# GuanLab/seekmer

Measured on AMD Instinct MI355X. Metric: paired reads/sec mapped+quantified, higher is better.
Workload: dtype u64+f64; 1 GPU; configs[1]: synthetic ~190k-tx index (stand-in for ENSEMBL GRCh38 cDNA), 10000000 2x100bp synthetic pairs per GPU, map+classes+EM to the reference stop rule; transcripts=190402, kmer_slots=134217728, units_per_gpu=10000000, read_len=100, paired=True, classes=851072, class_map_rows=4208693, parallelism=reads sharded x1, RCCL all-reduce f64[T] per EM step, rccl_ranks=0

## Files before the change

seekmer_amd/csrc/skm_abi.hip:

```cpp
#include "../../include/seekmer_hip.h"
#include "skm_kernels.h"
#include "skm_pool.h"
#include "skm_bias.h"
#include "skm_bias_weights.h"

#include <dlfcn.h>
#include <algorithm>
#include <cmath>
#include <cstdarg>
#include <cstdio>
#include <cstdlib>
#include <cstring>
#include <chrono>
#include <condition_variable>
#include <atomic>
#include <deque>
#include <functional>
#include <map>
#include <memory>
#include <unordered_map>
#include <mutex>
#include <thread>
#include <numeric>
#include <string>
// ... 3697 lines not shown
        aligned = q->pinned[32];
        q->n_total_reduced = true;
        if (const char *v = getenv("SKM_TEST_ALIGNED_GLOBAL")) aligned += strtoull(v, nullptr, 10);
    }
    q->n_total = (double)aligned;
    HIP_TRY(hipMemcpyAsync(q->x1.p, lengths, n_tx * 8, hipMemcpyHostToDevice, q->stream));
    if (m->use_length_weights)
        launch_effective_lengths_weights(m->length_weights.p, 1, q->x1.p, n_tx, q->eff_len.p, q->stream);
    else
        launch_effective_lengths(fld.p, q->x1.p, n_tx, q->eff_len.p, q->stream);
    if (q->comm ? aligned == 0 : C == 0) {
        if (effective_lengths)
            HIP_TRY(hipMemcpyAsync(effective_lengths, q->eff_len.p, n_tx * 8, hipMemcpyDeviceToHost, q->stream));
        HIP_TRY(hipStreamSynchronize(q->stream));
        if (tpm) memset(tpm, 0, (size_t)n_tx * 8);
        if (iters) *iters = 0;
        return SKM_OK;
    }
    launch_reciprocal(q->eff_len.p, n_tx, q->x0.p, q->stream);
    launch_np_sum(q->x0.p, n_tx, 1.0, sums.p, total, q->stream);
    launch_divide(q->x0.p, n_tx, total, false, 0.0, q->stream);
    lap("start vector");
    SKM_TRY(quant_finish_setup(q.get(), &m->t, m->first_seen_bound));
    lap("setup");
    if (trace) fprintf(stderr, "[skm_quant_infer] %lld classes, %lld transcripts, %lld rows\n", (long long)C, (long long)n_tx,
                       (long long)q->n_rows);
    int64_t it = 0;
    SKM_TRY(em_run(q.get(), rel_tol, x_floor, max_iters, 0, &it));
    lap("em");
    m->t_em_ns += q->t_em_ns;
    m->em_iters += (double)it;
    double *const x = (it & 1) ? q->x1.p : q->x0.p;
    launch_np_sum(x, n_tx, 1000000.0, sums.p, total, q->stream);
    launch_divide(x, n_tx, total + 1, true, 0.001, q->stream);
    launch_np_sum(x, n_tx, 1000000.0, sums.p, total, q->stream);
    launch_divide(x, n_tx, total + 1, false, 0.0, q->stream);
    HIP_TRY(hipGetLastError());
    if (tpm) HIP_TRY(hipMemcpyAsync(tpm, x, n_tx * 8, hipMemcpyDeviceToHost, q->stream));
    if (effective_lengths)
        HIP_TRY(hipMemcpyAsync(effective_lengths, q->eff_len.p, n_tx * 8, hipMemcpyDeviceToHost, q->stream));
    HIP_TRY(hipStreamSynchronize(q->stream));
    lap("tpm");
    if (iters) *iters = it;
    q.reset();
    lap("destroy");
    return SKM_OK;
}

extern "C" int skm_quant_destroy(skm_quant *q)
{
    if (!q) return SKM_OK;
    STALE_CHECK("quant_destroy entry");
    delete q;
    STALE_CHECK("quant_destroy exit");
    return SKM_OK;
}

extern "C" int skm_quant_em(skm_quant *q, double *x, const double *l, double rel_tol, double x_floor,
                            int64_t max_iters, int64_t fixed_iters, int64_t *iters)
{
    if (!q || !x || !l) return fail(SKM_ERR_ARG, "NULL argument");
    std::lock_guard<std::mutex> lock(q->mu);
    SKM_TRY(set_device(q->device));
    HIP_TRY(hipMemcpyAsync(q->x0.p, x, q->n_tx * 8, hipMemcpyHostToDevice, q->stream));
    HIP_TRY(hipMemcpyAsync(q->eff_len.p, l, q->n_tx * 8, hipMemcpyHostToDevice, q->stream));
    int64_t it = 0;
    SKM_TRY(em_run(q, rel_tol, x_floor, max_iters, fixed_iters, &it));
    HIP_TRY(hipMemcpy(x, (it & 1) ? q->x1.p : q->x0.p, q->n_tx * 8, hipMemcpyDeviceToHost));
    if (iters) *iters = it;
    return SKM_OK;
}

extern "C" int skm_quant_components(skm_quant *q, int64_t info[8], int32_t *tx_label, int32_t *tx_tile,
                                    int32_t *class_tile)
{
    if (!q || !info) return fail(SKM_ERR_ARG, "NULL argument");
    std::lock_guard<std::mutex> lock(q->mu);
    SKM_TRY(set_device(q->device));
    const auto &t = q->tiles;
    info[0] = t.built ? 1 : 0;
    info[1] = t.n_tiles;
    info[2] = t.n_oversize;
    info[3] = em_uses_tiles(q) ? 1 : 0;
    info[4] = EM_TILE_PAIRS; info[5] = EM_TILE_CLASSES; info[6] = EM_TILE_TX; info[7] = 0;
    if (!t.built) {
        if (tx_label || tx_tile || class_tile) return fail(SKM_ERR_ARG, "no component tiles were built for this handle");
        return SKM_OK;
    }
    HIP_TRY(hipStreamSynchronize(q->stream));
    if (tx_label) HIP_TRY(hipMemcpy(tx_label, t.tx_label.p, q->n_tx * 4, hipMemcpyDeviceToHost));
    if (tx_tile) HIP_TRY(hipMemcpy(tx_tile, t.tx_tile.p, q->n_tx * 4, hipMemcpyDeviceToHost));
    if (class_tile && q->n_classes) {
        std::vector<int32_t> tile(q->n_classes), perm(q->n_classes);
        HIP_TRY(hipMemcpy(tile.data(), t.cls_tile.p, q->n_classes * 4, hipMemcpyDeviceToHost));
        HIP_TRY(hipMemcpy(perm.data(), q->perm.p, q->n_classes * 4, hipMemcpyDeviceToHost));
        for (int64_t k = 0; k < q->n_classes; ++k) class_tile[perm[k]] = tile[k];
    }
    return SKM_OK;
}

extern "C" int skm_quant_set_counts(skm_quant *q, const double *class_counts)
{
    if (!q || (!class_counts && q->n_classes)) return fail(SKM_ERR_ARG, "NULL argument");
    std::lock_guard<std::mutex> lock(q->mu);
    SKM_TRY(set_device(q->device));
    const double total = np_sum_host(class_counts, q->n_classes);
    if (q->n_classes) {
        SKM_TRY(q->cls_count_saved.ensure(q->n_classes));
        HIP_TRY(hipMemcpyAsync(q->cls_count_saved.p, class_counts, q->n_classes * 8, hipMemcpyHostToDevice, q->stream));
        launch_permute_f64(q->cls_count_saved.p, q->perm.p, q->n_classes, q->cls_count.p, false, q->stream);
        HIP_TRY(hipGetLastError());
        HIP_TRY(hipStreamSynchronize(q->stream));
    }
    q->n_total = total;
    return SKM_OK;
}

namespace {

template <class Fill>
int em_group_run(skm_quant *q, int64_t n_problems, Fill &&fill, bool batched, int64_t slot_cap, const double *x0,
                 const double *l, double rel_tol, double x_floor, int64_t max_iters, double *out, int64_t *iters_out,
                 bool tpm)
{
    const int64_t C = q->n_classes, T = q->n_tx;
    skm_quant::Batch &w = q->batch;
    const int64_t group = std::max<int64_t>(1, std::min<int64_t>(n_problems, (int64_t)(1LL << 28) / T));
    const int64_t by_counts = std::max<int64_t>(1, (int64_t)((1LL << 31) / (8 * std::max<int64_t>(C, 1))));
    int64_t slots = batched ? std::max<int64_t>(1, std::min(group, by_counts)) : 1;
    if (slot_cap > 0) slots = std::min(slots, slot_cap);
    SKM_TRY(q->cls_count_saved.ensure(C));
    SKM_TRY(q->x_start.ensure(T));
    SKM_TRY(q->boot_out.ensure((size_t)(slots * T)));
    SKM_TRY(w.totals.ensure((size_t)(2 * slots)));
    HIP_TRY(hipMemcpyAsync(q->cls_count_saved.p, q->cls_count.p, C * 8, hipMemcpyDeviceToDevice, q->stream));
    HIP_TRY(hipMemcpyAsync(q->eff_len.p, l, T * 8, hipMemcpyHostToDevice, q->stream));
    HIP_TRY(hipMemcpyAsync(q->x_start.p, x0, T * 8, hipMemcpyHostToDevice, q->stream));
    const double saved_total = q->n_total;
    int rc = SKM_OK;
    DBuf<double> sums;
    auto restore = on_exit([&]() {
        (void)hipMemcpyAsync(q->cls_count.p, q->cls_count_saved.p, C * 8, hipMemcpyDeviceToDevice, q->stream);
        (void)hipStreamSynchronize(q->stream);
        q->n_total = saved_total;
    });
    auto problem_checked = [&](int64_t b, int64_t *it_out, double *dst) -> int {
        SKM_TRY(fill(b, (int64_t)1, q->cls_count.p, w.totals.p));
        HIP_TRY(hipGetLastError());
        double total = 0.0;
        HIP_TRY(hipMemcpyAsync(&total, w.totals.p, 8, hipMemcpyDeviceToHost, q->stream));
        HIP_TRY(hipMemcpyAsync(q->x0.p, q->x_start.p, T * 8, hipMemcpyDeviceToDevice, q->stream));
        HIP_TRY(hipStreamSynchronize(q->stream));
        q->n_total = total;
        SKM_TRY(em_run(q, rel_tol, x_floor, max_iters, 0, it_out, 8));
        HIP_TRY(hipMemcpyAsync(dst, (*it_out & 1) ? q->x1.p : q->x0.p, T * 8, hipMemcpyDeviceToDevice, q->stream));
        if (iters_out) iters_out[b] = *it_out;
        return SKM_OK;
    };
    auto scale = [&](double *results, int64_t count) -> int {
        if (!tpm || count <= 0) return SKM_OK;
        const int64_t n_blocks = (T + 8191) / 8192;
        SKM_TRY(sums.ensure((size_t)(count * (n_blocks + 2))));
        double *const totals = sums.p + count * n_blocks;
        launch_np_sum_many(results, T, count, T, 1000000.0, sums.p, totals, q->stream);
        launch_divide_many(results, T, count, T, totals + 1, true, 0.001, q->stream);
        launch_np_sum_many(results, T, count, T, 1000000.0, sums.p, totals, q->stream);
        launch_divide_many(results, T, count, T, totals + 1, false, 0.0, q->stream);
// ... 788 lines not shown
```

seekmer_amd/csrc/skm_kernels.h:

```cpp
#pragma once
#include "skm_device.h"

namespace skm {

struct MapBatch {
    const uint32_t *records;
    int64_t n_units;
    int32_t words_per_read;
    int32_t record_words;
    int32_t paired;
    int32_t *workspace;
    int32_t *rec_unit;
    uint64_t *rec_key;
    unsigned long long *rec_tuple;
    int32_t keep_spans;
    int32_t *unit_begin, *unit_end;
    Coord *unit_anchor;
    int32_t *unit_entries;
    int64_t ids_capacity;
    unsigned long long *ids_cursor;
    unsigned long long *fld;
    unsigned long long *stats;
    int32_t vote[8];
};
// ... 82 lines not shown
__host__ __device__ inline int tuple_len(long long t) { return (int)(t >> 40); }
struct ClassTable {
    ClassSlot *slots;
    uint64_t slot_mask;
    int32_t *arena;
    int64_t arena_capacity;
    unsigned long long *arena_cursor;
    unsigned long long *n_classes;
    unsigned long long *n_unaligned;
    unsigned long long *n_units;
    unsigned long long *global_fld;
    int64_t *class_list;
    int64_t class_list_capacity;
    unsigned long long *n_listed;
    unsigned long long *n_deferred;
    unsigned long long *arena_committed;
    int *error;
};
constexpr int CLASS_PROBE_LIMIT = 128;
void launch_class_insert(const ClassTable &t, const MapBatch &b, int64_t unit_base,
                         int64_t *unit_slot, bool retry_deferred, bool merge_fld, hipStream_t stream);
void launch_class_verify(const ClassTable &t, const MapBatch &b, const int64_t *unit_slot,
                         hipStream_t stream);
void launch_class_rehash(const ClassTable &from, const ClassTable &to, int64_t *forward,
                         hipStream_t stream);
void launch_slot_remap(int64_t *slots, int64_t n, const int64_t *forward, hipStream_t stream);
void launch_class_init(const ClassTable &t, hipStream_t stream);
void launch_class_compact(const ClassTable &t, int64_t n_classes, int64_t *cls_offset,
                          int64_t *cls_len, double *cls_count, unsigned long long *cls_first_seen,
                          hipStream_t stream);
void launch_class_merge(const ClassTable &t, int64_t n_classes, const int64_t *class_offsets,
                        const int32_t *class_targets, const int64_t *class_counts,
                        const int64_t *first_seen, hipStream_t stream);

void launch_class_merge_device(const ClassTable &t, int64_t n_classes, const int64_t *class_start,
                               const int64_t *class_len, const int32_t *ids, const double *class_counts,
                               const unsigned long long *first_seen, hipStream_t stream);
void launch_class_add_totals(const ClassTable &t, unsigned long long unaligned, unsigned long long units,
                             const unsigned long long *fld, hipStream_t stream);

constexpr int EM_ROW_CAP = 512;

struct EmProblem {
    int64_t n_tx, n_classes, n_rows;
    const int64_t *cls_offset;
    const int32_t *ids;
    const double *cls_count;
    double *inner;
    const int64_t *row_start;
    const int32_t *row_tx;
    const int32_t *tx_cls;
    const int64_t *tx_row;
    double *row_sum;
    const double *eff_len;
    double *x[2];
    double *acc;
    double n_total;
    double rel_tol, x_floor;
    unsigned long long *ctl;
    double *part_max;
    unsigned int *part_flags;
    int64_t max_iters, fixed_iters;
    int fused;
    unsigned int *arrivals;
    const double *extra_max;
    const unsigned int *extra_flags;
    int64_t n_extra, extra_first;
};
enum { CTL_DONE = 0, CTL_ITERS = 1, CTL_UNDEFINED = 3, CTL_TILE_FAULT = 4 };
#ifndef SKM_EM_FINAL_BLOCKS
#define SKM_EM_FINAL_BLOCKS 2048
#endif
constexpr int EM_FINAL_BLOCKS = SKM_EM_FINAL_BLOCKS;
void launch_em_inner(const EmProblem &p, int parity, bool judge_previous, int64_t steps_done, hipStream_t stream);
void launch_em_decide(const EmProblem &p, int64_t steps_done, hipStream_t stream);
void launch_em_rows(const EmProblem &p, int parity, hipStream_t stream);
void launch_em_rows_finalize(const EmProblem &p, int parity, hipStream_t stream);
void launch_em_rows_acc(const EmProblem &p, int parity, hipStream_t stream);
void launch_em_rows_to_acc(const EmProblem &p, hipStream_t stream);
void launch_em_finalize(const EmProblem &p, int parity, bool from_acc, hipStream_t stream);
void launch_em_result(const unsigned long long *ctl, const double *x0, const double *x1, int64_t n, double *out,
                      hipStream_t stream);

constexpr int EM_TILE_PAIRS = 2048, EM_TILE_CLASSES = 512, EM_TILE_TX = 128;
#ifndef SKM_EM_TILE_SEGMENT
#define SKM_EM_TILE_SEGMENT 128
#endif
constexpr int EM_TILE_SEGMENT = SKM_EM_TILE_SEGMENT;
constexpr int EM_CHUNK_MAX = 16;
constexpr int EM_TILE_CLASS_BATCH = 4;
struct EmTiles {
    int64_t n_tiles;
    const int64_t *tile_tx;
    const int64_t *tile_cls;
    const int32_t *tx_list;
    const int32_t *cls_list;
    const int64_t *cls_pair;
    const int64_t *tx_pair;
    const uint16_t *cls_tx;
    const uint16_t *tx_cls;
    double *step_max;
    unsigned int *step_flags;
    double *snap;
};
void launch_em_local_chunk(const EmProblem &p, const EmTiles &tiles, const double *x_in, int n_steps, int64_t first_step,
                           hipStream_t stream);
void launch_em_local_decide(const EmProblem &p, const EmTiles &tiles, int64_t first_step, int n_steps, hipStream_t stream);

constexpr int EM_BATCH = 8;
struct EmBatchProblem {
    int64_t n_tx, n_classes, n_rows;
    const int64_t *cls_offset;
    const int32_t *ids;
    const int64_t *row_start;
    const int32_t *row_tx;
    const int32_t *tx_cls;
    const int64_t *tx_row;
    const double *eff_len;
    const double *cls_count;
    double *inner;
    double *row_sum;
    double *x[2];
    double *place_total;
    double rel_tol, x_floor;
    unsigned long long *ctl;
    double *part_max;
    unsigned int *part_flags;
    int managed;
    unsigned long long *mgr;
    int64_t *iters_out;
    int fused;
    unsigned int *arrivals;
};
enum { BCTL_ALL_DONE = 0, BCTL_LAST_STEP = 1, BCTL_DONE = 8, BCTL_ITERS = 16, BCTL_UNDEFINED = 24 };
enum { MGR_NEXT = 0, MGR_COUNT = 1, MGR_FINISHED = 2, MGR_UNDEFINED = 3, MGR_REP = 8, MGR_SINCE = 16, MGR_TAKE = 24,
       MGR_PUT = 32 };
void launch_em_batch_manage_init(const EmBatchProblem &p, unsigned long long *mgr, unsigned long long *host_pinned64,
                                 int64_t n_reps, const double *counts_all, const double *totals, const double *x_start,
                                 double *out_all, hipStream_t stream);
void launch_em_batch_manage(const EmBatchProblem &p, unsigned long long *mgr, const double *counts_all, const double *totals,
                            const double *x_start, double *out_all, int64_t *iters_out, int64_t step, bool planned,
                            hipStream_t stream);
void launch_em_batch_step(const EmBatchProblem &p, int64_t step, hipStream_t stream);
void launch_em_batch_decide(const EmBatchProblem &p, int64_t steps_done, hipStream_t stream);
void launch_em_batch_take(const double *x, int64_t n_tx, int r, double *out, hipStream_t stream);
void launch_em_batch_ctl(unsigned long long *ctl, unsigned int idle, hipStream_t stream);
void launch_blend_counts(const double *own, const int32_t *class_cell, const double *weight, const double *cell_total,
                         int64_t n_cells, int64_t first, int64_t n_rows, int64_t n_classes, double *rows, hipStream_t stream);
void launch_permute_rows_f64(const double *x, const int32_t *perm, int64_t n, int64_t n_rows, double *y, hipStream_t stream);
struct EmSetSlot {
    int64_t cls_first, cls_end;
    int64_t row_first, row_end;
    double n_total;
    unsigned long long done;
    unsigned long long iters;
    unsigned long long undefined;
};
struct EmSetProblem {
    const int64_t *cls_offset;
    const int32_t *ids;
    const double *cls_count;
    double *inner;
    const int64_t *row_start;
    const int32_t *row_tx;
    const int32_t *tx_cls;
    const int64_t *tx_row;
    double *row_sum;
    const double *eff_len;
    double *x[2];
    double rel_tol, x_floor;
    int64_t max_iters;
// ... 96 lines not shown
```

seekmer_amd/csrc/skm_quant_setup.hip:

```cpp
#include "skm_kernels.h"
#include "skm_pool.h"

#include <algorithm>
#include <cstdio>
#include <vector>

namespace skm {

namespace {

struct Scratch {
    hipStream_t stream;
    std::vector<void *> held;
    explicit Scratch(hipStream_t s) : stream(s) {}
    template <class T>
    T *alloc(size_t n)
    {
        void *p = nullptr;
        if (pool_alloc(&p, std::max<size_t>(n, 1) * sizeof(T)) != hipSuccess) return nullptr;
        held.push_back(p);
        return static_cast<T *>(p);
    }
    ~Scratch()
    {
// ... 649 lines not shown
    }
    return v;
}

__global__ void __launch_bounds__(256)
cc_hook_kernel(const int64_t *cls_offset, const int32_t *ids, int64_t n_classes, int32_t *parent)
{
    for (int64_t c = blockIdx.x * (int64_t)blockDim.x + threadIdx.x; c < n_classes;
         c += (int64_t)gridDim.x * blockDim.x) {
        const int64_t begin = cls_offset[c], end = cls_offset[c + 1];
        if (begin == end) continue;
        int32_t b = cc_root_halving(parent, ids[begin]);
        for (int64_t j = begin + 1; j < end; ++j) {
            int32_t a = cc_root_halving(parent, ids[j]);
            while (a != b) {
                if (a < b) { const int32_t s = a; a = b; b = s; }
                const int32_t old = atomicCAS(&parent[a], a, b);
                if (old == a) break;
                a = cc_root_halving(parent, old);
            }
            b = a < b ? a : b;
        }
    }
}

__global__ void __launch_bounds__(256)
cc_label_kernel(int32_t *parent, const int64_t *tx_row, const int64_t *row_start, int64_t n_tx,
                int32_t *label, int32_t *comp)
{
    const int lane = threadIdx.x & 63;
    const int64_t stride = (int64_t)gridDim.x * blockDim.x;
    for (int64_t t0 = blockIdx.x * (int64_t)blockDim.x + threadIdx.x - lane; t0 < n_tx; t0 += stride) {
        const int64_t t = t0 + lane;
        int32_t r = -1, degree = 0;
        if (t < n_tx) {
            r = cc_root_halving(parent, (int32_t)t);
            label[t] = r;
            degree = (int32_t)(row_start[tx_row[t + 1]] - row_start[tx_row[t]]);
        }
        unsigned long long todo = __ballot(r >= 0);
        while (todo) {
            const int leader = __ffsll((long long)todo) - 1;
            const int32_t r0 = __shfl(r, leader, 64);
            const bool mine = r == r0;
            const unsigned long long same = __ballot(mine);
            int sum = mine ? degree : 0;
            for (int d = 32; d > 0; d >>= 1) sum += __shfl_xor(sum, d, 64);
            if (lane == leader) {
                atomicAdd(&comp[3 * (int64_t)r0], (int)__popcll(same));
                atomicAdd(&comp[3 * (int64_t)r0 + 1], sum);
            }
            todo &= ~same;
        }
    }
}

__global__ void __launch_bounds__(256)
cc_classes_kernel(const int64_t *cls_offset, const int32_t *ids, int64_t n_classes, const int32_t *label,
                  int32_t *comp)
{
    const int lane = threadIdx.x & 63;
    const int64_t stride = (int64_t)gridDim.x * blockDim.x;
    for (int64_t c0 = blockIdx.x * (int64_t)blockDim.x + threadIdx.x - lane; c0 < n_classes; c0 += stride) {
        const int64_t c = c0 + lane;
        int32_t r = -1;
        if (c < n_classes) {
            const int64_t begin = cls_offset[c];
            r = label[begin < cls_offset[c + 1] ? ids[begin] : 0];
        }
        const int32_t before = __shfl_up(r, 1, 64);
        const unsigned long long heads = __ballot(lane == 0 || before != r);
        if (r >= 0 && ((heads >> lane) & 1ULL)) {
            const unsigned long long later = lane == 63 ? 0ULL : heads >> (lane + 1);
            const int run = later ? __ffsll((long long)later) : 64 - lane;
            atomicAdd(&comp[3 * (int64_t)r + 2], run);
        }
    }
}

__global__ void __launch_bounds__(256)
tile_pack_kernel(const int32_t *__restrict__ comp, int64_t n_tx, int64_t n_segments, int32_t *__restrict__ root_tile,
                 int64_t *__restrict__ seg_tiles, unsigned long long *__restrict__ oversize)
{
    for (int64_t g = blockIdx.x * (int64_t)blockDim.x + threadIdx.x; g < n_segments;
         g += (int64_t)gridDim.x * blockDim.x) {
        int tx = 0, pairs = 0, classes = 0, n = 0;
        const int64_t last = min(n_tx, (g + 1) * EM_TILE_SEGMENT);
        for (int64_t t0 = g * EM_TILE_SEGMENT; t0 < last; t0 += 8) {
            int size[24];
#pragma unroll
            for (int k = 0; k < 24; ++k) size[k] = 3 * t0 + k < 3 * n_tx ? comp[3 * t0 + k] : 0;
#pragma unroll
            for (int k = 0; k < 8; ++k) {
                const int64_t t = t0 + k;
                if (t >= last) break;
                const int c_tx = size[3 * k], c_pairs = size[3 * k + 1], c_classes = size[3 * k + 2];
                if (c_tx == 0) { root_tile[t] = -1; continue; }
                if (c_tx > EM_TILE_TX || c_pairs > EM_TILE_PAIRS || c_classes > EM_TILE_CLASSES) {
                    root_tile[t] = -2;
                    atomicAdd(oversize, 1ULL);
                    continue;
                }
                if (n == 0 || tx + c_tx > EM_TILE_TX || pairs + c_pairs > EM_TILE_PAIRS ||
                    classes + c_classes > EM_TILE_CLASSES) {
                    ++n;
                    tx = pairs = classes = 0;
                }
                tx += c_tx; pairs += c_pairs; classes += c_classes;
                root_tile[t] = n - 1;
            }
        }
        seg_tiles[g] = n;
    }
}

__global__ void __launch_bounds__(256)
tx_tile_kernel(const int32_t *label, const int32_t *root_tile, const int64_t *seg_base, int64_t n_tx,
               const int64_t *tx_row, const int64_t *row_start, int degree_bits, int32_t *tx_tile, int32_t *key)
{
    for (int64_t t = blockIdx.x * (int64_t)blockDim.x + threadIdx.x; t < n_tx;
         t += (int64_t)gridDim.x * blockDim.x) {
        const int32_t r = label[t], at = root_tile[r];
        const int32_t tile = at < 0 ? (int32_t)n_tx : (int32_t)(seg_base[r / EM_TILE_SEGMENT] + at);
        tx_tile[t] = tile;
        const int64_t turns = (row_start[tx_row[t + 1]] - row_start[tx_row[t]] + 7) >> 3;
        const int32_t longest = (1 << degree_bits) - 1;
        key[t] = (tile << degree_bits) | (longest - (int32_t)min(turns, (int64_t)longest));
    }
}

#ifndef SKM_EM_CLASS_ORDER
#define SKM_EM_CLASS_ORDER 1
#endif
__global__ void __launch_bounds__(256)
cls_tile_kernel(const int64_t *cls_offset, const int32_t *ids, int64_t n_classes, const int32_t *tx_tile,
                int length_bits, int32_t *cls_tile, int32_t *key)
{
    for (int64_t c = blockIdx.x * (int64_t)blockDim.x + threadIdx.x; c < n_classes;
         c += (int64_t)gridDim.x * blockDim.x) {
        const int64_t begin = cls_offset[c], end = cls_offset[c + 1];
        const int32_t tile = tx_tile[begin < end ? ids[begin] : 0];
        cls_tile[c] = tile;
        const int64_t turns = (end - begin + EM_TILE_CLASS_BATCH - 1) / EM_TILE_CLASS_BATCH;
        const int32_t longest = (1 << length_bits) - 1;
        key[c] = (tile << length_bits) | (longest - (int32_t)min(turns, (int64_t)longest));
    }
}

__global__ void __launch_bounds__(256)
tile_starts_kernel(const int32_t *sorted_tile, int shift, int64_t n, const int64_t *n_tiles, int64_t *first)
{
    const int64_t tiles = *n_tiles;
    for (int64_t j = blockIdx.x * (int64_t)blockDim.x + threadIdx.x; j <= n;
         j += (int64_t)gridDim.x * blockDim.x) {
        const int64_t lo = j == 0 ? -1 : min((int64_t)(sorted_tile[j - 1] >> shift), tiles);
        const int64_t hi = j == n ? tiles : min((int64_t)(sorted_tile[j] >> shift), tiles);
        for (int64_t t = lo + 1; t <= hi; ++t) first[t] = j;
    }
}

__global__ void __launch_bounds__(256)
tile_local_tx_kernel(const int32_t *list, const int32_t *tile_sorted, int shift, const int64_t *first, const int64_t *n_tiles, int64_t n,
                     const int64_t *tx_row, const int64_t *row_start, int32_t *local, int64_t *len)
{
    for (int64_t i = blockIdx.x * (int64_t)blockDim.x + threadIdx.x; i < n;
         i += (int64_t)gridDim.x * blockDim.x) {
        const int32_t t = list[i];
        local[t] = (int32_t)(i - first[min((int64_t)(tile_sorted[i] >> shift), *n_tiles)]);
        len[i] = row_start[tx_row[t + 1]] - row_start[tx_row[t]];
    }
}

__global__ void __launch_bounds__(256)
tile_local_cls_kernel(const int32_t *list, const int32_t *tile_sorted, int shift, const int64_t *first, const int64_t *n_tiles, int64_t n,
                      const int64_t *cls_offset, int32_t *local, int64_t *len)
{
    for (int64_t k = blockIdx.x * (int64_t)blockDim.x + threadIdx.x; k < n;
         k += (int64_t)gridDim.x * blockDim.x) {
        const int32_t c = list[k];
        local[c] = (int32_t)(k - first[min((int64_t)(tile_sorted[k] >> shift), *n_tiles)]);
        len[k] = cls_offset[c + 1] - cls_offset[c];
    }
}

__global__ void __launch_bounds__(256)
tile_fill_cls_kernel(const int32_t *cls_list, int64_t n_classes, const int64_t *cls_offset, const int32_t *ids,
                     const int32_t *tx_local, const int64_t *cls_pair, const int32_t *cls_tile, int32_t residual_tile,
                     uint16_t *out)
{
    for (int64_t k = blockIdx.x * (int64_t)blockDim.x + threadIdx.x; k < n_classes;
         k += (int64_t)gridDim.x * blockDim.x) {
        const int32_t c = cls_list[k];
        if (cls_tile[c] == residual_tile) continue;
        const int64_t src = cls_offset[c], n = cls_offset[c + 1] - src, dst = cls_pair[k];
        for (int64_t j = 0; j < n; ++j) out[dst + j] = (uint16_t)tx_local[ids[src + j]];
    }
}

__global__ void __launch_bounds__(256)
tile_fill_tx_kernel(const int32_t *tx_list, int64_t n_tx, const int64_t *tx_row, const int64_t *row_start,
                    const int32_t *tx_cls, const int32_t *cls_local, const int64_t *tx_pair, const int32_t *tx_tile,
                    uint16_t *out)
{
    const int sub = threadIdx.x & 7;
    for (int64_t i = (blockIdx.x * (int64_t)blockDim.x + threadIdx.x) >> 3; i < n_tx;
         i += ((int64_t)gridDim.x * blockDim.x) >> 3) {
        const int32_t t = tx_list[i];
        if (tx_tile[t] == (int32_t)n_tx) continue;
        const int64_t src = row_start[tx_row[t]], n = row_start[tx_row[t + 1]] - src, dst = tx_pair[i];
        for (int64_t j = sub; j < n; j += 8) out[dst + j] = (uint16_t)cls_local[tx_cls[src + j]];
    }
}

int build_tiles(Scratch &scratch, QuantBuild &q)
{
    hipStream_t stream = scratch.stream;
    const int64_t C = q.n_classes, M = q.n_ids, T = q.n_tx;
    if (M >= (1LL << 31) || C >= (1LL << 31) || T >= (1LL << 31) - 2) return -2;
    const int64_t n_segments = (T + EM_TILE_SEGMENT - 1) / EM_TILE_SEGMENT;
    QB_ALLOC(parent, int32_t, T); QB_ALLOC(comp, int32_t, 3 * T); QB_ALLOC(root_tile, int32_t, T);
    QB_ALLOC(seg_tiles, int64_t, n_segments); QB_ALLOC(seg_base, int64_t, n_segments + 1);
    QB_ALLOC(oversize, unsigned long long, 1);
    QB_ALLOC(iota, int32_t, std::max(T, C)); QB_ALLOC(sorted_tile, int32_t, std::max(T, C));
    QB_ALLOC(tx_local, int32_t, T); QB_ALLOC(cls_local, int32_t, C);
    QB_ALLOC(len, int64_t, std::max(T, C));
    QB_TRY(hipMemsetAsync(comp, 0, 3 * T * sizeof(int32_t), stream));
    QB_TRY(hipMemsetAsync(oversize, 0, sizeof(unsigned long long), stream));
    hipLaunchKernelGGL(iota_kernel, dim3(blocks_for(T)), dim3(256), 0, stream, parent, T);
    hipLaunchKernelGGL(cc_hook_kernel, dim3(blocks_for(C)), dim3(256), 0, stream, q.cls_offset, q.ids, C, parent);
    hipLaunchKernelGGL(cc_label_kernel, dim3(blocks_for(T)), dim3(256), 0, stream, parent, q.tx_row, q.row_start, T,
                       q.tx_label, comp);
    hipLaunchKernelGGL(cc_classes_kernel, dim3(blocks_for(C)), dim3(256), 0, stream, q.cls_offset, q.ids, C,
                       q.tx_label, comp);
    hipLaunchKernelGGL(tile_pack_kernel, dim3(blocks_for(n_segments)), dim3(256), 0, stream, comp, T, n_segments,
                       root_tile, seg_tiles, oversize);
    if (exclusive_scan_with_total(scratch, seg_tiles, seg_base, n_segments)) return -1;
    int end_bit = 1;
    while ((1LL << end_bit) < T + 1 && end_bit < 31) ++end_bit;
    const int degree_bits = end_bit + 5 <= 31 ? 5 : 0;
    QB_ALLOC(tx_key, int32_t, T);
    hipLaunchKernelGGL(tx_tile_kernel, dim3(blocks_for(T)), dim3(256), 0, stream, q.tx_label, root_tile, seg_base, T,
                       q.tx_row, q.row_start, degree_bits, q.tx_tile, tx_key);
    hipLaunchKernelGGL(iota_kernel, dim3(blocks_for(std::max(T, C))), dim3(256), 0, stream, iota, std::max(T, C));
    if (sort_pairs(scratch, tx_key, sorted_tile, iota, q.tx_list, T, end_bit + degree_bits)) return -1;
    hipLaunchKernelGGL(tile_starts_kernel, dim3(blocks_for(T + 1)), dim3(256), 0, stream, sorted_tile, degree_bits, T,
                       seg_base + n_segments, q.tile_tx);
    hipLaunchKernelGGL(tile_local_tx_kernel, dim3(blocks_for(T)), dim3(256), 0, stream, q.tx_list, sorted_tile, degree_bits,
                       q.tile_tx, seg_base + n_segments, T, q.tx_row, q.row_start, tx_local, len);
    if (exclusive_scan_with_total(scratch, len, q.tx_pair, T)) return -1;
    const int length_bits = SKM_EM_CLASS_ORDER ? degree_bits : 0;
    QB_ALLOC(cls_key, int32_t, C);
    hipLaunchKernelGGL(cls_tile_kernel, dim3(blocks_for(C)), dim3(256), 0, stream, q.cls_offset, q.ids, C, q.tx_tile,
                       length_bits, q.cls_tile, cls_key);
    if (sort_pairs(scratch, cls_key, sorted_tile, iota, q.cls_list, C, end_bit + length_bits)) return -1;
    hipLaunchKernelGGL(tile_starts_kernel, dim3(blocks_for(C + 1)), dim3(256), 0, stream, sorted_tile, length_bits, C,
                       seg_base + n_segments, q.tile_cls);
    hipLaunchKernelGGL(tile_local_cls_kernel, dim3(blocks_for(C)), dim3(256), 0, stream, q.cls_list, sorted_tile, length_bits,
                       q.tile_cls, seg_base + n_segments, C, q.cls_offset, cls_local, len);
    if (exclusive_scan_with_total(scratch, len, q.cls_pair, C)) return -1;
    hipLaunchKernelGGL(tile_fill_cls_kernel, dim3(blocks_for(C)), dim3(256), 0, stream, q.cls_list, C, q.cls_offset,
                       q.ids, tx_local, q.cls_pair, q.cls_tile, (int32_t)T, q.tile_cls_tx);
    hipLaunchKernelGGL(tile_fill_tx_kernel, dim3(blocks_for(8 * T)), dim3(256), 0, stream, q.tx_list, T, q.tx_row,
                       q.row_start, q.tx_cls, cls_local, q.tx_pair, q.tx_tile, q.tile_tx_cls);
    QB_TRY(hipMemcpyAsync(&q.tile_info[0], seg_base + n_segments, sizeof(int64_t), hipMemcpyDeviceToHost, stream));
    QB_TRY(hipMemcpyAsync(&q.tile_info[1], oversize, sizeof(int64_t), hipMemcpyDeviceToHost, stream));
    return 0;
}

}

int64_t quant_setup(const ClassTable *table, QuantBuild &q, int32_t *perm, hipStream_t stream)
{
    const bool can_rank = table && q.first_seen_bound > 0 && q.first_seen_bound <= RANK_BITMAP_MAX_UNITS;
    for (int attempt = can_rank ? 0 : 1; attempt < 2; ++attempt) {
        int64_t n_rows = -1;
        {
            Scratch scratch(stream);
            if (attempt == 0) {
                const int rc = build_from_table_ranked(scratch, *table, q, perm);
                if (rc == 1) continue;
                if (rc) return -1;
            } else {
                if (table && build_from_table(scratch, *table, q)) return -1;
                if (localize(scratch, q, perm)) return -1;
            }
            if (transpose(scratch, q)) return -1;
            if (q.tile_tx && build_tiles(scratch, q)) return -1;
            QB_TRY(hipGetLastError());
            QB_TRY(hipMemcpyAsync(&n_rows, q.tx_row + q.n_tx, sizeof(int64_t), hipMemcpyDeviceToHost, stream));
        }
        if (n_rows > q.n_rows_cap) return -3;
        return n_rows;
    }
    return -1;
}

namespace {

__global__ void __launch_bounds__(256)
residual_count_kernel(const int32_t *cls_tile, const int64_t *cls_offset, int64_t n_classes, const int32_t *tx_tile,
                      const int64_t *tx_row, int64_t n_tx, unsigned long long *counts)
{
    unsigned long long classes = 0, pairs = 0, rows = 0;
    for (int64_t i = blockIdx.x * (int64_t)blockDim.x + threadIdx.x; i < max(n_classes, n_tx);
         i += (int64_t)gridDim.x * blockDim.x) {
        if (i < n_classes && cls_tile[i] == (int32_t)n_tx) { ++classes; pairs += cls_offset[i + 1] - cls_offset[i]; }
        if (i < n_tx && tx_tile[i] == (int32_t)n_tx) rows += tx_row[i + 1] - tx_row[i];
    }
    if (classes) atomicAdd(&counts[0], classes);
    if (pairs) atomicAdd(&counts[1], pairs);
    if (rows) atomicAdd(&counts[2], rows);
}

__global__ void __launch_bounds__(256)
residual_class_sizes_kernel(const int32_t *cls_tile, const int64_t *cls_offset, int64_t n_classes, int32_t residual_tile,
                            int64_t *keep, int64_t *len)
{
// ... 100 lines not shown
```

seekmer_amd/infer.py:

```python
import ctypes
import datetime
import json
import logging
import os
import pathlib
import shlex
import sys

import numpy

from . import _native
from . import common
from . import mapper

__all__ = ['run', 'run_many', 'gene_map', 'gene_sums', 'gene_unique_counts', 'gene_table', 'bias_correct', 'bias_pass', 'bias_correct_many', 'bias_pass_many', 'quantify', 'quantify_many', 'quantify_tables', 'quantify_resident', 'em', 'output_results', 'bootstrap_quantify',
           'bootstrap_ranks']

_LOG = logging.getLogger(__name__)

REL_TOL = 0.01
X_FLOOR = 1e-8


def run(index_path, output_path, fastq_paths, job_count, save_readmap,
# ... 482 lines not shown
def _feeder(fastq_paths, paired, parse_threads, shard, keep_reference_batches, sum_over_ranks=None):
    import os
    cores = len(os.sched_getaffinity(0)) if hasattr(os, 'sched_getaffinity') else (os.cpu_count() or 1)
    total = 0
    for path in fastq_paths:
        try:
            total += os.path.getsize(str(path))
        except OSError:
            pass
    one_rank = shard is None or shard[1] <= 1
    if (one_rank or sum_over_ranks is not None) and not keep_reference_batches and parse_threads != 0 \
            and common.PackedReadFeeder.eligible(fastq_paths):
        threads = parse_threads if parse_threads else max(1, min(16, cores - 1))
        world = 1 if one_rank else shard[1]
        return common.PackedReadFeeder(fastq_paths, paired, threads=threads, pinned=total > (1 << 30) * world,
                                       shard=None if one_rank else shard, sum_over_ranks=sum_over_ranks)
    if parse_threads is None:
        parse_threads = 0 if keep_reference_batches else min(8, cores)
    if parse_threads <= 0:
        return common.NativeReadFeeder(fastq_paths, paired=paired, shard=shard)
    return common.NativeReadFeeder(fastq_paths, paired=paired, batch_units=1 << (20 if total > (16 << 30) else 18),
                                   threads=parse_threads, pinned=total > (4 << 30), shard=shard)


def finish(map_result, ranks, quantify_ranks, comm=None):
    from . import parallel
    if ranks.world == 1:
        summarized = map_result.summarize()
        _LOG.info('Quantifying transcripts')
        return summarized, quantify(summarized)
    _LOG.info('Quantifying transcripts')
    tpm = quantify_ranks(map_result)
    import os
    if comm and os.environ.get('SKM_HANDOVER') == 'rccl':
        parallel.hand_over_device(map_result, comm, ranks)
        return (map_result.summarize() if ranks.rank == 0 else None), tpm
    tables = ranks.gather_arrays_to_root(parallel.rank_table(map_result) if ranks.rank else {})
    if ranks.rank != 0:
        return None, tpm
    parallel.merge_into(map_result, tables[1:])
    return map_result.summarize(), tpm


class _QuantHandle:

    def __init__(self, handle, n_tx, n_classes):
        self.handle = handle
        self.n_tx = n_tx
        self.n_classes = n_classes

    @classmethod
    def from_csr(cls, n_tx, offsets, targets, counts, device=0):
        offsets = numpy.ascontiguousarray(offsets, dtype=numpy.int64)
        targets = numpy.ascontiguousarray(targets if len(targets) else [0], dtype=numpy.int32)
        counts = numpy.ascontiguousarray(counts if len(counts) else [0.0], dtype='f8')
        out = ctypes.c_void_p()
        _native.check(_native.hip().skm_quant_create(
            device, n_tx, offsets.size - 1, _native.ptr(offsets, _native.c_i64p),
            _native.ptr(targets, _native.c_i32p), _native.ptr(counts, _native.c_f64p),
            ctypes.byref(out)))
        return cls(out, n_tx, offsets.size - 1)

    @classmethod
    def from_map_result(cls, map_result, n_tx):
        out = ctypes.c_void_p()
        _native.check(_native.hip().skm_quant_create_from_mapper(
            map_result._handle, n_tx, ctypes.byref(out)))
        return cls(out, n_tx, map_result.sizes()[0])

    def em(self, x, l, fixed_iters=0, max_iters=0, rel_tol=REL_TOL, x_floor=X_FLOOR):
        x = numpy.array(x, dtype='f8', copy=True, order='C')
        l = numpy.ascontiguousarray(l, dtype='f8')
        iters = ctypes.c_int64()
        _native.check(_native.hip().skm_quant_em(
            self.handle, _native.ptr(x, _native.c_f64p), _native.ptr(l, _native.c_f64p),
            rel_tol, x_floor, max_iters, fixed_iters, ctypes.byref(iters)))
        return x, iters.value

    def components(self, arrays=True):
        raw = numpy.zeros(8, dtype=numpy.int64)
        _native.check(_native.hip().skm_quant_components(self.handle, _native.ptr(raw, _native.c_i64p),
                                                         None, None, None))
        info = {'built': bool(raw[0]), 'tiles': int(raw[1]), 'oversize': int(raw[2]), 'em_uses_tiles': bool(raw[3]),
                'capacity': (int(raw[4]), int(raw[5]), int(raw[6]))}
        if not arrays or not info['built']:
            return info, None, None, None
        label = numpy.zeros(self.n_tx, dtype=numpy.int32)
        tile = numpy.zeros(self.n_tx, dtype=numpy.int32)
        class_tile = numpy.zeros(max(self.n_classes, 1), dtype=numpy.int32)
        _native.check(_native.hip().skm_quant_components(
            self.handle, _native.ptr(raw, _native.c_i64p), _native.ptr(label, _native.c_i32p),
            _native.ptr(tile, _native.c_i32p), _native.ptr(class_tile, _native.c_i32p)))
        return info, label, tile, class_tile[:self.n_classes]

    def set_counts(self, counts):
        counts = numpy.ascontiguousarray(counts, dtype='f8')
        _native.check(_native.hip().skm_quant_set_counts(self.handle,
                                                         _native.ptr(counts, _native.c_f64p)))

    def bootstrap(self, n_boot, seed, x0, l, want_counts=False, tpm=False):
        x0 = numpy.ascontiguousarray(x0, dtype='f8')
        l = numpy.ascontiguousarray(l, dtype='f8')
        out = numpy.zeros((n_boot, self.n_tx), dtype='f8')
        if tpm and not want_counts:
            iters = numpy.zeros(max(n_boot, 1), dtype=numpy.int64)
            _native.check(_native.hip().skm_quant_bootstrap_tpm(
                self.handle, n_boot, seed, _native.ptr(x0, _native.c_f64p),
                _native.ptr(l, _native.c_f64p), REL_TOL, X_FLOOR, 0,
                _native.ptr(out, _native.c_f64p), _native.ptr(iters, _native.c_i64p)))
            return out, None, iters[:n_boot]
        counts = numpy.zeros((n_boot, max(self.n_classes, 1)), dtype=numpy.int64) if want_counts else None
        iters = numpy.zeros(max(n_boot, 1), dtype=numpy.int64)
        _native.check(_native.hip().skm_quant_bootstrap(
            self.handle, n_boot, seed, _native.ptr(x0, _native.c_f64p),
            _native.ptr(l, _native.c_f64p), REL_TOL, X_FLOOR, 0,
            _native.ptr(out, _native.c_f64p),
            _native.ptr(counts, _native.c_i64p) if want_counts else None,
            _native.ptr(iters, _native.c_i64p)))
        return out, counts, iters[:n_boot]

    def em_many(self, counts, x0, l, tpm=False):
        counts = numpy.ascontiguousarray(counts, dtype='f8')
        if counts.ndim != 2 or counts.shape[1] != self.n_classes:
            raise ValueError('counts must be [K, %d]' % self.n_classes)
        x0 = numpy.ascontiguousarray(x0, dtype='f8')
        l = numpy.ascontiguousarray(l, dtype='f8')
        n = counts.shape[0]
        out = numpy.zeros((n, self.n_tx), dtype='f8')
        iters = numpy.zeros(max(n, 1), dtype=numpy.int64)
        _native.check(_native.hip().skm_quant_em_many(
            self.handle, n, _native.ptr(counts, _native.c_f64p), _native.ptr(x0, _native.c_f64p),
            _native.ptr(l, _native.c_f64p), REL_TOL, X_FLOOR, int(bool(tpm)), _native.ptr(out, _native.c_f64p),
            _native.ptr(iters, _native.c_i64p)))
        return out, iters[:n]

    def em_blend(self, class_cell, weight, cell_total, x0, l, tpm=False, want_counts=False):
        class_cell = numpy.ascontiguousarray(class_cell, dtype=numpy.int32)
        weight = numpy.ascontiguousarray(weight, dtype='f8')
        cell_total = numpy.ascontiguousarray(cell_total, dtype='f8')
        n = cell_total.size
        if weight.shape != (n, n) or class_cell.size != self.n_classes:
            raise ValueError('weight must be [n, n] and class_cell [C] for n = len(cell_total) cells')
        x0 = numpy.ascontiguousarray(x0, dtype='f8')
        l = numpy.ascontiguousarray(l, dtype='f8')
        out = numpy.zeros((n, self.n_tx), dtype='f8')
        iters = numpy.zeros(max(n, 1), dtype=numpy.int64)
        counts = numpy.zeros((n, max(self.n_classes, 1)), dtype='f8') if want_counts else None
        _native.check(_native.hip().skm_quant_em_blend(
            self.handle, n, _native.ptr(class_cell, _native.c_i32p), _native.ptr(weight, _native.c_f64p),
            _native.ptr(cell_total, _native.c_f64p), _native.ptr(x0, _native.c_f64p), _native.ptr(l, _native.c_f64p),
            REL_TOL, X_FLOOR, int(bool(tpm)), _native.ptr(out, _native.c_f64p), _native.ptr(iters, _native.c_i64p),
            _native.ptr(counts, _native.c_f64p) if want_counts else None))
        return out, iters[:n], (counts[:, :self.n_classes] if want_counts else None)

    def timing(self):
        out = (ctypes.c_double * 4)()
        _native.check(_native.hip().skm_quant_timing(self.handle, out))
        return {'em_ns': out[0], 'iterations': int(out[1]), 'launches': int(out[2])}

    def close(self):
        if self.handle:
            _native.hip().skm_quant_destroy(self.handle)
            self.handle = None

    def __del__(self):
        try:
            self.close()
# ... 448 lines not shown
```

Before: 969.9 million pairs/s.

## Pack EM component tiles with a wave-parallel scan instead of one thread per segment

The tile packing kernel now assigns one 64-lane wave per segment instead of one thread. It computes prefix sums of transcript, pair and class counts with shuffles and finds tile break points by ballot, which replaces the serial per-thread greedy loop. The default packing segment grows from 128 to 256 transcripts, and the tile capacities become compile-time overridable. The greedy tile boundaries should match the serial version, and the larger segment may change tile counts slightly. The break-finding loop iterates once per tile opened within each 64-transcript chunk.

```diff
diff --git a/seekmer_amd/csrc/skm_abi.hip b/seekmer_amd/csrc/skm_abi.hip
--- a/seekmer_amd/csrc/skm_abi.hip
+++ b/seekmer_amd/csrc/skm_abi.hip
@@ -3803,7 +3803,7 @@
     info[1] = t.n_tiles;
     info[2] = t.n_oversize;
     info[3] = em_uses_tiles(q) ? 1 : 0;
-    info[4] = EM_TILE_PAIRS; info[5] = EM_TILE_CLASSES; info[6] = EM_TILE_TX; info[7] = 0;
+    info[4] = EM_TILE_PAIRS; info[5] = EM_TILE_CLASSES; info[6] = EM_TILE_TX; info[7] = EM_TILE_SEGMENT;
     if (!t.built) {
         if (tx_label || tx_tile || class_tile) return fail(SKM_ERR_ARG, "no component tiles were built for this handle");
         return SKM_OK;
diff --git a/seekmer_amd/csrc/skm_kernels.h b/seekmer_amd/csrc/skm_kernels.h
--- a/seekmer_amd/csrc/skm_kernels.h
+++ b/seekmer_amd/csrc/skm_kernels.h
@@ -188,11 +188,22 @@
 void launch_em_result(const unsigned long long *ctl, const double *x0, const double *x1, int64_t n, double *out,
                       hipStream_t stream);
 
-constexpr int EM_TILE_PAIRS = 2048, EM_TILE_CLASSES = 512, EM_TILE_TX = 128;
+#ifndef SKM_EM_TILE_PAIRS
+#define SKM_EM_TILE_PAIRS 2048
+#endif
+#ifndef SKM_EM_TILE_CLASSES
+#define SKM_EM_TILE_CLASSES 512
+#endif
+#ifndef SKM_EM_TILE_TX
+#define SKM_EM_TILE_TX 128
+#endif
 #ifndef SKM_EM_TILE_SEGMENT
-#define SKM_EM_TILE_SEGMENT 128
-#endif
+#define SKM_EM_TILE_SEGMENT 256
+#endif
+constexpr int EM_TILE_PAIRS = SKM_EM_TILE_PAIRS, EM_TILE_CLASSES = SKM_EM_TILE_CLASSES, EM_TILE_TX = SKM_EM_TILE_TX;
+static_assert(EM_TILE_PAIRS <= 65535 && EM_TILE_CLASSES <= 65535 && EM_TILE_TX <= 65535, "tile-local indices and offsets are 16 bits wide");
 constexpr int EM_TILE_SEGMENT = SKM_EM_TILE_SEGMENT;
+static_assert(EM_TILE_SEGMENT > 0, "a packing run holds at least one transcript id");
 constexpr int EM_CHUNK_MAX = 16;
 constexpr int EM_TILE_CLASS_BATCH = 4;
 struct EmTiles {
diff --git a/seekmer_amd/csrc/skm_quant_setup.hip b/seekmer_amd/csrc/skm_quant_setup.hip
--- a/seekmer_amd/csrc/skm_quant_setup.hip
+++ b/seekmer_amd/csrc/skm_quant_setup.hip
@@ -755,35 +755,48 @@
 tile_pack_kernel(const int32_t *__restrict__ comp, int64_t n_tx, int64_t n_segments, int32_t *__restrict__ root_tile,
                  int64_t *__restrict__ seg_tiles, unsigned long long *__restrict__ oversize)
 {
-    for (int64_t g = blockIdx.x * (int64_t)blockDim.x + threadIdx.x; g < n_segments;
-         g += (int64_t)gridDim.x * blockDim.x) {
+    const int lane = threadIdx.x & 63;
+    const int64_t n_waves = ((int64_t)gridDim.x * blockDim.x) >> 6;
+    for (int64_t g = (blockIdx.x * (int64_t)blockDim.x + threadIdx.x) >> 6; g < n_segments; g += n_waves) {
         int tx = 0, pairs = 0, classes = 0, n = 0;
         const int64_t last = min(n_tx, (g + 1) * EM_TILE_SEGMENT);
-        for (int64_t t0 = g * EM_TILE_SEGMENT; t0 < last; t0 += 8) {
-            int size[24];
-#pragma unroll
-            for (int k = 0; k < 24; ++k) size[k] = 3 * t0 + k < 3 * n_tx ? comp[3 * t0 + k] : 0;
-#pragma unroll
-            for (int k = 0; k < 8; ++k) {
-                const int64_t t = t0 + k;
-                if (t >= last) break;
-                const int c_tx = size[3 * k], c_pairs = size[3 * k + 1], c_classes = size[3 * k + 2];
-                if (c_tx == 0) { root_tile[t] = -1; continue; }
-                if (c_tx > EM_TILE_TX || c_pairs > EM_TILE_PAIRS || c_classes > EM_TILE_CLASSES) {
-                    root_tile[t] = -2;
-                    atomicAdd(oversize, 1ULL);
-                    continue;
-                }
-                if (n == 0 || tx + c_tx > EM_TILE_TX || pairs + c_pairs > EM_TILE_PAIRS ||
-                    classes + c_classes > EM_TILE_CLASSES) {
-                    ++n;
-                    tx = pairs = classes = 0;
-                }
-                tx += c_tx; pairs += c_pairs; classes += c_classes;
-                root_tile[t] = n - 1;
+        for (int64_t t0 = g * EM_TILE_SEGMENT; t0 < last; t0 += 64) {
+            const int64_t t = t0 + lane;
+            int c_tx = 0, c_pairs = 0, c_classes = 0;
+            if (t < last) { c_tx = comp[3 * t]; c_pairs = comp[3 * t + 1]; c_classes = comp[3 * t + 2]; }
+            const bool root = c_tx > 0;
+            const bool big = c_tx > EM_TILE_TX || c_pairs > EM_TILE_PAIRS || c_classes > EM_TILE_CLASSES;
+            const bool packed = root && !big;
+            if (!packed) c_tx = c_pairs = c_classes = 0;
+            int s_tx = c_tx, s_pairs = c_pairs, s_classes = c_classes;
+            for (int d = 1; d < 64; d <<= 1) {
+                const int a = __shfl_up(s_tx, d, 64), b = __shfl_up(s_pairs, d, 64), c = __shfl_up(s_classes, d, 64);
+                if (lane >= d) { s_tx += a; s_pairs += b; s_classes += c; }
             }
-        }
-        seg_tiles[g] = n;
+            int base_tx = -tx, base_pairs = -pairs, base_classes = -classes, opened = 0;
+            const int before = n;
+            unsigned long long behind = ~0ULL;
+            for (;;) {
+                const bool over = packed && (n == 0 || s_tx - base_tx > EM_TILE_TX || s_pairs - base_pairs > EM_TILE_PAIRS ||
+                                             s_classes - base_classes > EM_TILE_CLASSES);
+                const unsigned long long starts = __ballot(over) & behind;
+                if (!starts) break;
+                const int at = __ffsll((long long)starts) - 1;
+                base_tx = __shfl(s_tx - c_tx, at, 64);
+                base_pairs = __shfl(s_pairs - c_pairs, at, 64);
+                base_classes = __shfl(s_classes - c_classes, at, 64);
+                ++n;
+                if (lane >= at) ++opened;
+                behind = at == 63 ? 0ULL : ~0ULL << (at + 1);
+            }
+            if (t < last) root_tile[t] = !root ? -1 : big ? -2 : before + opened - 1;
+            const unsigned long long bigs = __ballot(root && big);
+            if (bigs && lane == 0) atomicAdd(oversize, (unsigned long long)__popcll(bigs));
+            tx = __shfl(s_tx, 63, 64) - base_tx;
+            pairs = __shfl(s_pairs, 63, 64) - base_pairs;
+            classes = __shfl(s_classes, 63, 64) - base_classes;
+        }
+        if (lane == 0) seg_tiles[g] = n;
     }
 }
 
@@ -905,7 +918,7 @@
                        q.tx_label, comp);
     hipLaunchKernelGGL(cc_classes_kernel, dim3(blocks_for(C)), dim3(256), 0, stream, q.cls_offset, q.ids, C,
                        q.tx_label, comp);
-    hipLaunchKernelGGL(tile_pack_kernel, dim3(blocks_for(n_segments)), dim3(256), 0, stream, comp, T, n_segments,
+    hipLaunchKernelGGL(tile_pack_kernel, dim3(blocks_for(64 * n_segments)), dim3(256), 0, stream, comp, T, n_segments,
                        root_tile, seg_tiles, oversize);
     if (exclusive_scan_with_total(scratch, seg_tiles, seg_base, n_segments)) return -1;
     int end_bit = 1;
diff --git a/seekmer_amd/infer.py b/seekmer_amd/infer.py
--- a/seekmer_amd/infer.py
+++ b/seekmer_amd/infer.py
@@ -588,7 +588,7 @@
         _native.check(_native.hip().skm_quant_components(self.handle, _native.ptr(raw, _native.c_i64p),
                                                          None, None, None))
         info = {'built': bool(raw[0]), 'tiles': int(raw[1]), 'oversize': int(raw[2]), 'em_uses_tiles': bool(raw[3]),
-                'capacity': (int(raw[4]), int(raw[5]), int(raw[6]))}
+                'capacity': (int(raw[4]), int(raw[5]), int(raw[6])), 'segment': int(raw[7])}
         if not arrays or not info['built']:
             return info, None, None, None
         label = numpy.zeros(self.n_tx, dtype=numpy.int32)
```

New measurement: 1.000 billion pairs/s, median of 6. 3.1% higher.
